# flxrcz/hommx

Hardware: AMD Instinct MI355X
Metric: micro-cell solves/sec (higher is better)
Workload: dtype f64

## Files before the change

### hommx_amd/csrc/fused2d.hip

```cpp
#include <hip/hip_runtime.h>
#include <stdint.h>

#include <type_traits>

#include "kernels.h"
#include "sweep_acc.h"

#ifndef HOMMX_FUSED_WAVES_PER_SIMD
#define HOMMX_FUSED_WAVES_PER_SIMD 2
#endif

namespace hommx {

typedef double d4 __attribute__((ext_vector_type(4)));
typedef double d2 __attribute__((ext_vector_type(2)));

__device__ __forceinline__ double uniform_f64(double v) {
  return __hiloint2double(__builtin_amdgcn_readfirstlane(__double2hiint(v)),
                          __builtin_amdgcn_readfirstlane(__double2loint(v)));
}

struct CoefRow {
  double a0, a1;
  double a0m, a1m;
};

constexpr int MATP = 48;

template <int NB>
struct alignas(16) Lds {
  double mat[(NB + 1) * MATP];
  double ubuf[4 * NB];
  double tsc[16 * 17];
  double rrow[2][NB];
  double vrow[2][NB];
  double vnat[2][NB];
  double e0row[NB];
  double e1row[NB];
  double e0nat[NB];
  double e1nat[NB];
  double dgnat[NB];
  double cenat[NB + 2];
};

struct NoFact {};
template <int NB, bool FACT>
__global__ __launch_bounds__(64, HOMMX_FUSED_WAVES_PER_SIMD) void k_poisson2d_fused(
    const double* __restrict__ coef, const double* __restrict__ Mmat, double* __restrict__ out,
    int32_t* __restrict__ info, int n, long long ncells, const CoefSource src, std::conditional_t<FACT, double*, NoFact> fact
#ifdef HOMMX_FUSED_DEBUG
    , double* __restrict__ dbg
#endif
) {
  constexpr int NT = NB / 16, KK = NB / 4, CG = 64 / NB;
  constexpr int P = MATP;
  __shared__ Lds<NB> L;

  const long long cell = blockIdx.x;
  if (cell >= ncells) return;
  __builtin_assume(n >= 3);
  __builtin_assume(n <= NB);
  const int l = threadIdx.x;
  const int j = l & 15, k = l >> 4;
  const int c = l % NB, g = l / NB;
  const int lb = l - c;
  const int p0 = NB - n;
  const bool valid = c >= p0;
  const int cn = c - p0;
  const int cm = valid ? (c == p0 ? NB - 1 : c - 1) : c;
  const int cp = valid ? (c == NB - 1 ? p0 : c + 1) : c;
  const int prow = (c & 3) * KK + (c >> 2);

  const int ownB = (k + 1) * P + j;
  int leftB[NT];
#pragma unroll
  for (int tj = 0; tj < NT; ++tj) {
    const int col = 16 * tj + j;
    leftB[tj] = (k + 1) * P + (col == p0 ? NB - 1 : col - 1);
  }
#define OWN(ti, tj, r) (ownB + (16 * (ti) + 4 * (r)) * P + 16 * (tj))
#define LEFT(ti, tj, r) (leftB[tj] + (16 * (ti) + 4 * (r)) * P)
  const unsigned matOff = accl::lds_offset(&L.mat[0]);
  const unsigned haloA = matOff + 8u * (unsigned)(p0 * P + j);

  const int mode = src.mode;
  const unsigned char* mask = static_cast<const unsigned char*>(src.table);
  const double* table = static_cast<const double*>(src.table);
  const double* cc = mode == COEF_STREAM ? coef + cell * (2ll * n * n) : coef + cell * 2;
  constexpr int NL = NB * NB / 64;
  double2 pv[NL];
  if (mode == COEF_STREAM) {
#pragma unroll
    for (int i = 0; i < NL; ++i) {
      const int el = 2 * l + 128 * i;
      pv[i] = el < 2 * n * n ? *reinterpret_cast<const double2*>(cc + el) : double2{0.0, 0.0};
    }
  }

  for (int i = l; i < (NB + 1) * P; i += 64) L.mat[i] = 0.0;
  if (l == 0) L.cenat[0] = 0.0;

  double m00 = 1.0, m01 = 0.0, m10 = 0.0, m11 = 1.0;
  if (Mmat) {
    const double* mp = Mmat + cell * 4;
    m00 = mp[0]; m01 = mp[1]; m10 = mp[2]; m11 = mp[3];
  }
  const double al = uniform_f64(0.5 * (m00 * m00 + m10 * m10));
  const double be = uniform_f64(0.5 * (m01 * m01 + m11 * m11));
  const double ga = uniform_f64(0.5 * (m00 * m01 + m10 * m11));
  const double ab = uniform_f64(al - 2.0 * ga + be);

  double ph0 = 0.0, ph1 = 0.0;
  if (mode != COEF_STREAM) {
    ph0 = cc[0];
    ph1 = cc[1];
  }
  const int nq = src.nq;
  auto sample = [&](long long el) {
    double acc = 0.0;
    for (int q = 0; q < nq; ++q)
      acc = add_rn(acc, mul_rn(src.weights[q], div_rn(1.0, add_rn(ph0, mul_rn(ph1, table[el * nq + q])))));
    return acc;
  };
  auto load_pair = [&](long long el, double& a0, double& a1) {
    if (mode == COEF_TWO_PHASE) {
      const uchar2 mk = *reinterpret_cast<const uchar2*>(mask + el);
      a0 = mk.x ? ph1 : ph0;
      a1 = mk.y ? ph1 : ph0;
    } else if (mode == COEF_AFFINE) {
      const double2 g2 = *reinterpret_cast<const double2*>(table + el);
      a0 = add_rn(ph0, mul_rn(ph1, g2.x));
      a1 = add_rn(ph0, mul_rn(ph1, g2.y));
    } else if (mode == COEF_RECIPROCAL) {
      a0 = sample(el);
      a1 = sample(el + 1);
    } else {
      const double2 v = *reinterpret_cast<const double2*>(cc + el);
      a0 = v.x; a1 = v.y;
    }
  };
  int esh;
  {
    int ef = 0;
    if (mode == COEF_STREAM) {
      int hm = 0;
#pragma unroll
      for (int i = 0; i < NL; ++i) hm = max(hm, max(__double2hiint(pv[i].x) & 0x7fffffff, __double2hiint(pv[i].y) & 0x7fffffff));
      ef = hm >> 20;
    } else {
      for (long long el = 2 * l; el < 2ll * n * n; el += 128) {
        double a0, a1;
        load_pair(el, a0, a1);
        const int f0 = (__double2hiint(a0) >> 20) & 0x7ff, f1 = (__double2hiint(a1) >> 20) & 0x7ff;
        ef = max(ef, max(f0, f1));
      }
    }
#pragma unroll
    for (int off = 32; off >= 1; off >>= 1) ef = max(ef, __shfl_xor(ef, off, 64));
    const int fm = (__double2hiint(6.0 * (al + be)) >> 20) & 0x7ff;
    const int sh = (ef == 0 || ef == 0x7ff ? 0 : ef - 1023) + (fm == 0 || fm == 0x7ff ? 0 : fm - 1023) + 2;
    esh = __builtin_amdgcn_readfirstlane(ef == 0 || ef == 0x7ff ? 0 : sh);
  }
  auto load_row = [&](int jc) {
    CoefRow r;
    r.a0 = 0.0; r.a1 = 0.0;
    if (valid) {
      load_pair(2 * (jc * n + cn), r.a0, r.a1);
      r.a0 = ldexp(r.a0, -esh);
      r.a1 = ldexp(r.a1, -esh);
    }
    r.a0m = __shfl(r.a0, lb + cm, 64);
    r.a1m = __shfl(r.a1, lb + cm, 64);
    return r;
  };
  auto st_diag = [&](const CoefRow& cur, const CoefRow& prev) {
    return valid ? cur.a0 * al + cur.a1 * be + cur.a0m * ab + prev.a0m * be + prev.a1m * al + prev.a1 * ab : 1.0;
  };
  auto st_E = [&](const CoefRow& cur, const CoefRow& prev) { return (cur.a0 + prev.a1) * (ga - al); };
  auto st_N = [&](const CoefRow& cur) { return (cur.a1 + cur.a0m) * (ga - be); };
  auto st_NE = [&](const CoefRow& cur) { return -ga * (cur.a0 + cur.a1); };
  auto st_p0 = [&](const CoefRow& cur, const CoefRow& prev) { return cur.a0 - cur.a0m - prev.a1m + prev.a1; };
  auto st_p1 = [&](const CoefRow& cur, const CoefRow& prev) { return cur.a1 + cur.a0m - prev.a0m - prev.a1; };

  auto band_write = [&](double dv, double ov, bool sym, bool clear) {
    if (g == 0) {
      const double d_ = clear ? 0.0 : dv, o_ = clear ? 0.0 : ov;
      L.mat[(c + 1) * P + c] = d_;
      if (valid) {
        L.mat[(cp + 1) * P + c] = o_;
        if (sym) L.mat[(c + 1) * P + cp] = o_;
      }
    }
  };

  [[maybe_unused]] double* rec = nullptr;
  if constexpr (FACT) rec = fact + cell * fused_fact_doubles(n);
  [[maybe_unused]] double* srec = nullptr;
  if constexpr (FACT) srec = rec + fused_fact_header(NB);

  double wf[NT][KK];
  double a[NT][NT][4];
  d4 slr[NT][NT];
  double rr[2];
  double rlm;
  CoefRow cur;
  double asum;
  __syncthreads();
  {
    const CoefRow rowA = load_row(n - 2);
    const CoefRow rowB = load_row(n - 1);
    cur = load_row(0);
    asum = (rowB.a0 + rowB.a1) + (cur.a0 + cur.a1);
    if constexpr (FACT) {
      const double neB = st_NE(rowB);
      const double c1 = __shfl(neB, lb + cm, 64);
      if (g == 0) {
        rec[c] = st_N(rowB);
        rec[NB + c] = c1;
      }
      if (l < 4) rec[4 * NB + l] = l == 0 ? m00 : l == 1 ? m01 : l == 2 ? m10 : m11;
      if (l == 4) rec[4 * NB + 4] = (double)esh;
    }
    {
      const double dv = st_diag(rowB, rowA), ov = st_E(rowB, rowA);
      band_write(dv, ov, true, false);
      __syncthreads();
#pragma unroll
      for (int ti = 0; ti < NT; ++ti)
#pragma unroll
        for (int tj = 0; tj <= ti; ++tj)
#pragma unroll
          for (int r = 0; r < 4; ++r) slr[ti][tj][r] = L.mat[OWN(ti, tj, r)];
      __syncthreads();
      band_write(dv, ov, true, true);
      __syncthreads();
    }
    {
      const double dv = st_N(rowB), ov = st_NE(rowB);
      band_write(dv, ov, false, false);
      __syncthreads();
#pragma unroll
      for (int t = 0; t < NT; ++t)
#pragma unroll
        for (int kk = 0; kk < KK; ++kk) wf[t][kk] = L.mat[OWN(kk >> 2, t, kk & 3)];
      __syncthreads();
      band_write(dv, ov, false, true);
      __syncthreads();
    }
    {
      const double dv = -st_diag(cur, rowB), ov = -st_E(cur, rowB);
      band_write(dv, ov, true, false);
      __syncthreads();
#pragma unroll
      for (int ti = 0; ti < NT; ++ti)
#pragma unroll
        for (int tj = 0; tj < NT; ++tj)
#pragma unroll
          for (int r = 0; r < 4; ++r) a[ti][tj][r] = L.mat[OWN(ti, tj, r)];
      __syncthreads();
      band_write(dv, ov, true, true);
      __syncthreads();
    }
    rr[0] = st_p0(cur, rowB); rr[1] = st_p1(cur, rowB);
    rlm = (k >> 1) ? st_p1(rowB, rowA) : st_p0(rowB, rowA);
  }
  double ga_ = 0.0, gb_ = 0.0;
  int bad = 0, badstep = 0;
  double wselR[NT];
#pragma unroll
  for (int tj = 0; tj < NT; ++tj) wselR[tj] = (k == 3 && 16 * tj + j == p0) ? 1.0 : 0.0;
  const double wselC = (j == 15 && k == (p0 & 3)) ? 1.0 : 0.0;
  double indw[KK];
#pragma unroll
  for (int q = 0; q < KK; ++q) indw[q] = uniform_f64((q == (p0 >> 2)) ? 1.0 : 0.0);

  for (int jr = 0; jr <= n - 2; ++jr) {
    const bool lastStep = (jr == n - 2);
    CoefRow nxt = cur;
    if (!lastStep) {
      nxt = load_row(jr + 1);
      asum += nxt.a0 + nxt.a1;
    }
    const double e0c = st_N(cur);
    const double neC = st_NE(cur);
    const double e1c = __shfl(neC, lb + cm, 64);
    if (lastStep) {
      for (int i = l; i < (NB + 1) * P; i += 64) L.mat[i] = 0.0;
      __syncthreads();
      if (g == 0) {
        L.mat[(c + 1) * P + c] = e0c;
        if (valid) L.mat[(c + 1) * P + cp] = neC;
      }
      __syncthreads();
#pragma unroll
      for (int t = 0; t < NT; ++t)
#pragma unroll
        for (int kk = 0; kk < KK; ++kk) wf[t][kk] += L.mat[OWN(kk >> 2, t, kk & 3)];
      __syncthreads();
    }
    const double dgc = st_diag(nxt, cur), cec = st_E(nxt, cur);
    if (g == 0) {
      L.rrow[0][prow] = rr[0];
      L.rrow[1][prow] = rr[1];
      L.e0row[prow] = e0c;
      L.e1row[prow] = e1c;
      L.e0nat[c] = e0c;
      L.e1nat[c] = e1c;
      L.dgnat[c] = dgc;
      L.cenat[1 + c] = cec;
    }

    {
      int badj = 0;
#ifdef HOMMX_FUSED_SWEEP32
      accl::Sweep<NB>::run(a, L.ubuf, j, k, badj);
#else
      __builtin_amdgcn_s_setprio(1);
      if constexpr (NB == 32) accl::block_inverse32(a, L.ubuf, L.tsc, j, k, badj);
      else accl::Sweep<NB>::run(a, L.ubuf, j, k, badj);
      __builtin_amdgcn_s_setprio(0);
#endif
      if (badj && !bad) { bad = 1; badstep = jr + 1; }
    }
    if constexpr (FACT) {
#pragma unroll
      for (int ti = 0; ti < NT; ++ti)
#pragma unroll
        for (int tj = 0; tj < NT; ++tj)
#pragma unroll
          for (int r = 0; r < 4; ++r) srec[((ti * NT + tj) * 4 + r) * 64 + l] = a[ti][tj][r];
      if (g == 0) {
        srec[NB * NB + 2 * NB + c] = e0c;
        srec[NB * NB + 3 * NB + c] = e1c;
      }
    }
#ifdef HOMMX_FUSED_DEBUG
    if (dbg && cell == 0) {
      double* q = dbg + (size_t)jr * 4 * NB * NB;
#pragma unroll
      for (int ti = 0; ti < NT; ++ti)
#pragma unroll
        for (int tj = 0; tj < NT; ++tj)
#pragma unroll
          for (int r = 0; r < 4; ++r) q[(16 * ti + 4 * r + k) * NB + 16 * tj + j] = a[ti][tj][r];
#pragma unroll
      for (int t = 0; t < NT; ++t)
#pragma unroll
        for (int kk = 0; kk < KK; ++kk) q[NB * NB + (16 * t + j) * NB + 4 * kk + k] = wf[t][kk];
    }
#endif

    if (!lastStep) {
#pragma unroll
      for (int ti = 0; ti < NT; ++ti)
#pragma unroll
        for (int tj = 0; tj < NT; ++tj)
#pragma unroll
          for (int r = 0; r < 4; ++r) L.mat[OWN(ti, tj, r)] = a[ti][tj][r];
#pragma unroll
      for (int tj = 0; tj < NT; ++tj)
        accl::masked_lds_store<accl::RowMask<3>::lo, accl::RowMask<3>::hi>(haloA + 128u * tj, a[NT - 1][tj][3]);
    }

    d4 vt[NT][NT];
#pragma unroll
    for (int x = 0; x < NT; ++x)
#pragma unroll
      for (int y = 0; y < NT; ++y) vt[x][y] = d4{0.0, 0.0, 0.0, 0.0};
#pragma unroll
    for (int kk = 0; kk < KK; ++kk)
#pragma unroll
      for (int x = 0; x < NT; ++x)
#pragma unroll
        for (int y = 0; y < NT; ++y)
          vt[x][y] = __builtin_amdgcn_mfma_f64_16x16x4f64(a[kk >> 2][x][kk & 3], wf[y][kk], vt[x][y], 0, 0, 0);

#pragma unroll
    for (int kk = 0; kk < KK; ++kk)
#pragma unroll
      for (int x = 0; x < NT; ++x)
#pragma unroll
        for (int y = 0; y <= x; ++y)
          slr[x][y] = __builtin_amdgcn_mfma_f64_16x16x4f64(vt[kk >> 2][x][kk & 3], wf[y][kk], slr[x][y], 0, 0, 0);

    double z;
    {
      double part[2][NT];
#pragma unroll
      for (int m = 0; m < 2; ++m)
#pragma unroll
        for (int tj = 0; tj < NT; ++tj) part[m][tj] = 0.0;
#pragma unroll
      for (int m = 0; m < 2; ++m)
#pragma unroll
        for (int ti = 0; ti < NT; ++ti) {
          const d4 q = *reinterpret_cast<const d4*>(&L.rrow[m][k * KK + 4 * ti]);
#pragma unroll
          for (int r = 0; r < 4; ++r)
#pragma unroll
            for (int tj = 0; tj < NT; ++tj) part[m][tj] = fma(q[r], a[ti][tj][r], part[m][tj]);
        }
      if (NT == 2) {
        double s_[2];
#pragma unroll
        for (int m = 0; m < 2; ++m) {
          double x = part[m][0], y = part[m][NT - 1];
          swap16(x, y);
          s_[m] = x + y;
        }
        swap32(s_[0], s_[1]);
        z = s_[0] + s_[1];
      } else {
        double x = part[0][0], y = part[1][0];
        swap32(x, y);
        z = add_xor16(x + y);
      }
    }
    ga_ = fma(z, rr[0], ga_);
    gb_ = fma(z, rr[1], gb_);
    L.vnat[k >> 1][c] = z;
    L.vrow[k >> 1][prow] = z;
    if constexpr (FACT) {
      if (NB == 32 || !(k & 1)) srec[NB * NB + (k >> 1) * NB + c] = z;
      srec += fused_fact_step(NB);
    }

    {
      double part[2][NT];
#pragma unroll
      for (int m = 0; m < 2; ++m) {
        double v[KK];
#pragma unroll
        for (int q4 = 0; q4 < KK; q4 += 4) {
          const d4 q = *reinterpret_cast<const d4*>(&L.vrow[m][k * KK + q4]);
          v[q4] = q[0]; v[q4 + 1] = q[1]; v[q4 + 2] = q[2]; v[q4 + 3] = q[3];
        }
#pragma unroll
        for (int t = 0; t < NT; ++t) {
          double acc = 0.0;
#pragma unroll
          for (int kk = 0; kk < KK; ++kk) acc = fma(v[kk], wf[t][kk], acc);
          part[m][t] = acc;
        }
      }
      double z6;
      if (NT == 2) {
        double s_[2];
#pragma unroll
        for (int m = 0; m < 2; ++m) {
          double x = part[m][0], y = part[m][NT - 1];
          swap16(x, y);
          s_[m] = x + y;
        }
        swap32(s_[0], s_[1]);
        z6 = s_[0] + s_[1];
      } else {
        double x = part[0][0], y = part[1][0];
        swap32(x, y);
        z6 = add_xor16(x + y);
      }
      rlm += z6;
    }

    if (!lastStep) {
      double e0r[KK], e1r[KK];
#pragma unroll
      for (int q4 = 0; q4 < KK; q4 += 4) {
        const d4 x = *reinterpret_cast<const d4*>(&L.e0row[k * KK + q4]);
        const d4 y = *reinterpret_cast<const d4*>(&L.e1row[k * KK + q4]);
        e0r[q4] = x[0]; e0r[q4 + 1] = x[1]; e0r[q4 + 2] = x[2]; e0r[q4 + 3] = x[3];
        e1r[q4] = y[0]; e1r[q4 + 1] = y[1]; e1r[q4 + 2] = y[2]; e1r[q4 + 3] = y[3];
      }
      {
        double e0q[NT], e1q[NT], dgq[NT], ceq[NT], cemq[NT];
#pragma unroll
        for (int tj = 0; tj < NT; ++tj) {
          e0q[tj] = L.e0nat[16 * tj + j];
          e1q[tj] = L.e1nat[16 * tj + j];
          dgq[tj] = L.dgnat[16 * tj + j];
          ceq[tj] = L.cenat[1 + 16 * tj + j];
          cemq[tj] = L.cenat[16 * tj + j];
        }
#pragma unroll
        for (int ti = 0; ti < NT; ++ti)
#pragma unroll
          for (int r = 0; r < 4; ++r)
#pragma unroll
            for (int tj = 0; tj < NT; ++tj) {
              const double nl = L.mat[LEFT(ti, tj, r)];
              const double nu = L.mat[OWN(ti, tj, r) - P];
              const double nul = L.mat[LEFT(ti, tj, r) - P];
              const double x = fma(e1q[tj], nl, e0q[tj] * a[ti][tj][r]);
              const double xu = fma(e1q[tj], nul, e0q[tj] * nu);
              a[ti][tj][r] = -fma(e0r[4 * ti + r], x, e1r[4 * ti + r] * xu);
            }
#pragma unroll
        for (int t = 0; t < NT; ++t) {
          using namespace accl;
#define DIAG_LO(r) (OneLane<0, 4 * (r)>::lo | OneLane<1, 4 * (r) + 1>::lo | OneLane<2, 4 * (r) + 2>::lo | OneLane<3, 4 * (r) + 3>::lo)
#define DIAG_HI(r) (OneLane<0, 4 * (r)>::hi | OneLane<1, 4 * (r) + 1>::hi | OneLane<2, 4 * (r) + 2>::hi | OneLane<3, 4 * (r) + 3>::hi)
          masked_sub4<DIAG_LO(0), DIAG_HI(0), DIAG_LO(1), DIAG_HI(1), DIAG_LO(2), DIAG_HI(2), DIAG_LO(3), DIAG_HI(3)>(
              a[t][t][0], a[t][t][1], a[t][t][2], a[t][t][3], dgq[t]);
#define SUB_LO(r) (((r) ? OneLane<0, (4 * (r) - 1) & 15>::lo : 0u) | OneLane<1, 4 * (r)>::lo | OneLane<2, 4 * (r) + 1>::lo | OneLane<3, 4 * (r) + 2>::lo)
#define SUB_HI(r) (((r) ? OneLane<0, (4 * (r) - 1) & 15>::hi : 0u) | OneLane<1, 4 * (r)>::hi | OneLane<2, 4 * (r) + 1>::hi | OneLane<3, 4 * (r) + 2>::hi)
          masked_sub4<SUB_LO(0), SUB_HI(0), SUB_LO(1), SUB_HI(1), SUB_LO(2), SUB_HI(2), SUB_LO(3), SUB_HI(3)>(
              a[t][t][0], a[t][t][1], a[t][t][2], a[t][t][3], ceq[t]);
#define SUP_LO(r) (OneLane<0, 4 * (r) + 1>::lo | OneLane<1, 4 * (r) + 2>::lo | OneLane<2, 4 * (r) + 3>::lo | ((r) < 3 ? OneLane<3, (4 * (r) + 4) & 15>::lo : 0u))
#define SUP_HI(r) (OneLane<0, 4 * (r) + 1>::hi | OneLane<1, 4 * (r) + 2>::hi | OneLane<2, 4 * (r) + 3>::hi | ((r) < 3 ? OneLane<3, (4 * (r) + 4) & 15>::hi : 0u))
          masked_sub4<SUP_LO(0), SUP_HI(0), SUP_LO(1), SUP_HI(1), SUP_LO(2), SUP_HI(2), SUP_LO(3), SUP_HI(3)>(
              a[t][t][0], a[t][t][1], a[t][t][2], a[t][t][3], cemq[t]);
#undef DIAG_LO
#undef DIAG_HI
#undef SUB_LO
#undef SUB_HI
#undef SUP_LO
#undef SUP_HI
        }
        if (NT == 2) {
          using namespace accl;
          masked_sub<OneLane<0, 15>::lo, OneLane<0, 15>::hi>(a[NT - 1][0][0], ceq[0]);
          masked_sub<OneLane<3, 0>::lo, OneLane<3, 0>::hi>(a[0][NT - 1][3], cemq[NT - 1]);
        }
        {
          const double cw = readlane_f64(cec, NB - 1);
#pragma unroll
          for (int tj = 0; tj < NT; ++tj) a[NT - 1][tj][3] = fma(-cw, wselR[tj], a[NT - 1][tj][3]);
          const double vcol = -cw * wselC;
#pragma unroll
          for (int ti = 0; ti < NT; ++ti)
#pragma unroll
            for (int r = 0; r < 4; ++r) a[ti][NT - 1][r] = fma(vcol, indw[4 * ti + r], a[ti][NT - 1][r]);
        }
      }

#pragma unroll
      for (int x = 0; x < NT; ++x)
#pragma unroll
        for (int y = 0; y < NT; ++y)
#pragma unroll
          for (int r = 0; r < 4; ++r) L.mat[OWN(x, y, r)] = vt[x][y][r];
#pragma unroll
      for (int y = 0; y < NT; ++y)
        accl::masked_lds_store<accl::RowMask<3>::lo, accl::RowMask<3>::hi>(haloA + 128u * y, vt[NT - 1][y][3]);
#pragma unroll
      for (int t = 0; t < NT; ++t)
#pragma unroll
        for (int kk = 0; kk < KK; ++kk) {
          const double up = L.mat[OWN(kk >> 2, t, kk & 3) - P];
          wf[t][kk] = fma(e1r[kk], up, e0r[kk] * vt[kk >> 2][t][kk & 3]);
        }

      {
        const double v0 = L.vnat[0][c], v1 = L.vnat[1][c];
        const double vm0 = L.vnat[0][cm], vm1 = L.vnat[1][cm];
        rr[0] = fma(vm0, e1c, fma(v0, e0c, st_p0(nxt, cur)));
        rr[1] = fma(vm1, e1c, fma(v1, e0c, st_p1(nxt, cur)));
      }
      cur = nxt;
      __syncthreads();
    }
  }

  {
    if (NT == 2) {
#pragma unroll
      for (int r = 0; r < 4; ++r) L.mat[OWN(1, 0, r)] = slr[NT - 1][0][r];
      __syncthreads();
    }
#pragma unroll
    for (int ti = 0; ti < NT; ++ti)
#pragma unroll
      for (int tj = 0; tj < NT; ++tj)
#pragma unroll
        for (int r = 0; r < 4; ++r) {
          if (tj <= ti) a[ti][tj][r] = -slr[ti][tj][r];
          else a[ti][tj][r] = -L.mat[(16 + j + 1) * P + 4 * r + k];
        }
    {
      using namespace accl;
#pragma unroll
      for (int tj = 0; tj < NT; ++tj) amov<RowMask<3>::lo, RowMask<3>::hi>(a[NT - 1][tj][3], 0.0);
#pragma unroll
      for (int ti = 0; ti < NT; ++ti)
#pragma unroll
        for (int r = 0; r < 4; ++r) amov<ColMask<15>::lo, ColMask<15>::hi>(a[ti][NT - 1][r], 0.0);
      amov<OneLane<3, 15>::lo, OneLane<3, 15>::hi>(a[NT - 1][NT - 1][3], -1.0);
    }
    if (c == NB - 1) rlm = 0.0;
    __syncthreads();
    L.rrow[k >> 1][prow] = rlm;
    L.vnat[k >> 1][c] = rlm;
    __syncthreads();
    int badj = 0;
    accl::Sweep<NB>::run(a, L.ubuf, j, k, badj);
    if (badj && !bad) { bad = 1; badstep = n; }
    if constexpr (FACT) {
#pragma unroll
      for (int ti = 0; ti < NT; ++ti)
#pragma unroll
        for (int tj = 0; tj < NT; ++tj)
#pragma unroll
          for (int r = 0; r < 4; ++r) srec[((ti * NT + tj) * 4 + r) * 64 + l] = a[ti][tj][r];
    }
    double part[2][NT];
#pragma unroll
    for (int m = 0; m < 2; ++m)
#pragma unroll
      for (int tj = 0; tj < NT; ++tj) part[m][tj] = 0.0;
#pragma unroll
    for (int m = 0; m < 2; ++m)
#pragma unroll
      for (int ti = 0; ti < NT; ++ti) {
        const d4 q = *reinterpret_cast<const d4*>(&L.rrow[m][k * KK + 4 * ti]);
#pragma unroll
        for (int r = 0; r < 4; ++r)
#pragma unroll
          for (int tj = 0; tj < NT; ++tj) part[m][tj] = fma(q[r], a[ti][tj][r], part[m][tj]);
      }
    double z;
    if (NT == 2) {
      double s_[2];
#pragma unroll
      for (int m = 0; m < 2; ++m) {
        double x = part[m][0], y = part[m][NT - 1];
        swap16(x, y);
        s_[m] = x + y;
      }
      swap32(s_[0], s_[1]);
      z = s_[0] + s_[1];
    } else {
      double x = part[0][0], y = part[1][0];
      swap32(x, y);
      z = add_xor16(x + y);
    }
    ga_ = fma(z, L.vnat[0][c], ga_);
    gb_ = fma(z, L.vnat[1][c], gb_);
    if constexpr (FACT) {
      if (NB == 32 || !(k & 1)) rec[2 * NB + (k >> 1) * NB + c] = z;
    }
  }

  double g00 = (k < 2) ? ga_ : 0.0, g01 = (k < 2) ? gb_ : 0.0, g11 = (k < 2) ? 0.0 : gb_;
#pragma unroll
  for (int off = 32; off >= 1; off >>= 1) {
    g00 += __shfl_xor(g00, off, 64);
    g01 += __shfl_xor(g01, off, 64);
    g11 += __shfl_xor(g11, off, 64);
    asum += __shfl_xor(asum, off, 64);
  }
  if (l == 0) {
    const double h = 1.0 / n;
    constexpr int DUP = 32 / NB;
    const double sc = 0.25 * h * h / DUP;
    const double c0 = 0.5 * h * h * asum / CG;
    const double t00 = m00 * g00 + m01 * g01, t01 = m00 * g01 + m01 * g11;
    const double t10 = m10 * g00 + m11 * g01, t11 = m10 * g01 + m11 * g11;
    double* o = out + cell * 4;
    o[0] = ldexp(c0 + sc * (t00 * m00 + t01 * m01), esh);
    o[1] = ldexp(sc * (t00 * m10 + t01 * m11), esh);
    o[2] = ldexp(sc * (t10 * m00 + t11 * m01), esh);
    o[3] = ldexp(c0 + sc * (t10 * m10 + t11 * m11), esh);
    if (info) info[cell] = bad ? badstep : 0;
  }
#undef OWN
#undef LEFT
}

#ifndef HOMMX_FUSED_FACT_TU
hipError_t launch_poisson2d_fused(const double* d_coef, const double* d_M, double* d_out, int32_t* d_info,
                                  int n, long long ncells, hipStream_t stream, CoefSource src) {
  if (ncells <= 0) return hipSuccess;
  dim3 grid((unsigned)ncells), block(64);
#ifndef HOMMX_DEV_LDS_PAD
#define HOMMX_DEV_LDS_PAD 0
#endif
#ifdef HOMMX_FUSED_DEBUG
  extern double* g_fused_dbg;
  if (n <= 16)
    hipLaunchKernelGGL((k_poisson2d_fused<16, false>), grid, block, 0, stream, d_coef, d_M, d_out, d_info, n, ncells, src, NoFact{}, g_fused_dbg);
  else
    hipLaunchKernelGGL((k_poisson2d_fused<32, false>), grid, block, 0, stream, d_coef, d_M, d_out, d_info, n, ncells, src, NoFact{}, g_fused_dbg);
#else
  if (n <= 16)
    hipLaunchKernelGGL((k_poisson2d_fused<16, false>), grid, block, HOMMX_DEV_LDS_PAD, stream, d_coef, d_M, d_out, d_info, n, ncells, src, NoFact{});
  else
    hipLaunchKernelGGL((k_poisson2d_fused<32, false>), grid, block, HOMMX_DEV_LDS_PAD, stream, d_coef, d_M, d_out, d_info, n, ncells, src, NoFact{});
#endif
  return hipGetLastError();
}

#else
hipError_t launch_poisson2d_fused_fact(const double* d_coef, const double* d_M, double* d_out, int32_t* d_info, int n, long long ncells,
                                       hipStream_t stream, double* d_fact) {
  if (ncells <= 0) return hipSuccess;
  dim3 grid((unsigned)ncells), block(64);
  const CoefSource src;
#ifdef HOMMX_FUSED_DEBUG
  extern double* g_fused_dbg;
  if (n <= 16)
    hipLaunchKernelGGL((k_poisson2d_fused<16, true>), grid, block, 0, stream, d_coef, d_M, d_out, d_info, n, ncells, src, d_fact, g_fused_dbg);
  else
    hipLaunchKernelGGL((k_poisson2d_fused<32, true>), grid, block, 0, stream, d_coef, d_M, d_out, d_info, n, ncells, src, d_fact, g_fused_dbg);
#else
  if (n <= 16)
    hipLaunchKernelGGL((k_poisson2d_fused<16, true>), grid, block, 0, stream, d_coef, d_M, d_out, d_info, n, ncells, src, d_fact);
  else
    hipLaunchKernelGGL((k_poisson2d_fused<32, true>), grid, block, 0, stream, d_coef, d_M, d_out, d_info, n, ncells, src, d_fact);
#endif
  return hipGetLastError();
}
#endif

}
```

### hommx_amd/csrc/kernels.h

```cpp
#pragma once
#include <hip/hip_runtime.h>
#include <stdint.h>

#include <type_traits>

#include "../../include/hommx_hip.h"

namespace hommx {

struct KindSizes {
  int bs, t, n_comp;
};
constexpr KindSizes kind_sizes(int dim, int kind) {
  const int te = dim * (dim + 1) / 2;
  return kind == HOMMX_KIND_POISSON_SCALAR   ? KindSizes{1, dim, 1}
         : kind == HOMMX_KIND_POISSON_MATRIX ? KindSizes{1, dim, te}
         : kind == HOMMX_KIND_ELASTICITY_ISO ? KindSizes{dim, te, 2}
                                             : KindSizes{dim, te, te * (te + 1) / 2};
}

template <typename F>
auto dispatch_dim_kind(int dim, int kind, F&& f) {
  auto with_dim = [&](auto D) {
    switch (kind) {
      case 0: return f(D, std::integral_constant<int, 0>{});
      case 1: return f(D, std::integral_constant<int, 1>{});
      case 2: return f(D, std::integral_constant<int, 2>{});
      default: return f(D, std::integral_constant<int, 3>{});
    }
  };
  return dim == 2 ? with_dim(std::integral_constant<int, 2>{}) : with_dim(std::integral_constant<int, 3>{});
}

__device__ __forceinline__ double mul_rn(double a, double b) {
#pragma clang fp contract(off)
  return a * b;
}
__device__ __forceinline__ double add_rn(double a, double b) {
#pragma clang fp contract(off)
  return a + b;
}
__device__ __forceinline__ double div_rn(double a, double b) {
#pragma clang fp contract(off)
  return a / b;
}
enum CoefMode { COEF_STREAM = 0, COEF_TWO_PHASE = 1, COEF_AFFINE = 2, COEF_RECIPROCAL = 3 };
struct CoefSource {
  int mode = COEF_STREAM;
  int nq = 0;
  const void* table = nullptr;
  const double* weights = nullptr;
};

hipError_t launch_poisson2d_fused(const double* d_coef, const double* d_M, double* d_out, int32_t* d_info,
                                  int n, long long ncells, hipStream_t stream, CoefSource src = CoefSource());

constexpr long long fused_fact_header(int NB) { return 4 * NB + 8; }
constexpr long long fused_fact_step(int NB) { return (long long)NB * NB + 4 * NB; }
constexpr long long fused_fact_doubles(int n) {
  return fused_fact_header(n <= 16 ? 16 : 32) + (n - 1) * fused_fact_step(n <= 16 ? 16 : 32) + (n <= 16 ? 16 * 16 : 32 * 32);
}
hipError_t launch_poisson2d_fused_fact(const double* d_coef, const double* d_M, double* d_out, int32_t* d_info, int n, long long ncells,
                                       hipStream_t stream, double* d_fact);
hipError_t launch_fused2d_subst(const double* d_fact, double* d_corr, int n, long long ncells, hipStream_t stream);
hipError_t launch_fused2d_subst_rhs(const double* d_fact, const double* d_P, int n_loads, bool per_cell, const double* d_M, double* d_corr, int n,
                                    long long ncells, hipStream_t stream);

hipError_t launch_expand_separable(CoefSource src, const double* d_params, double* d_coef, long long n_el, int n_comp, long long ncells,
                                   hipStream_t stream);

hipError_t launch_expand_two_phase(const unsigned char* d_mask, const double* d_values, double* d_coef, long long n_el,
                                   int n_comp, long long ncells, hipStream_t stream);

struct ReconArgs {
  int n = 0;
  double vol_struct = 0.0;
  long long ndof = 0, n_el = 0;
  const int32_t* el_nodes = nullptr;
  const double* grads = nullptr;
  const double* vol = nullptr;
  const double* corr = nullptr;
  const double* coef = nullptr;
  const double* M = nullptr;
  const double* xi = nullptr;
  double* stats = nullptr;
  double* strain = nullptr;
  double* flux = nullptr;
  double* slot = nullptr;
  int n_regions = 0;
  const uint8_t* region = nullptr;
  double* region_stats = nullptr;
};
size_t recon_lds_limit();
hipError_t launch_reconstruct(const ReconArgs& a, int dim, int kind, bool mesh, long long nc, hipStream_t stream);

struct SensArgs {
  int n = 0;
  double vol_struct = 0.0;
  long long ndof = 0, n_el = 0;
  const int32_t* el_nodes = nullptr;
  const double* grads = nullptr;
  const double* vol = nullptr;
  const double* corr = nullptr;
  const double* M = nullptr;
  int n_dirs = 0;
  bool per_cell = false;
  const double* dirs = nullptr;
  double* dA = nullptr;
  const double* weights = nullptr;
  double* grad = nullptr;
};
hipError_t launch_sensitivity(const SensArgs& a, int dim, int kind, bool mesh, long long nc, hipStream_t stream);

struct LoadArgs {
  int n = 0;
  double vol_struct = 0.0;
  long long ndof = 0, n_el = 0;
  const int32_t* el_nodes = nullptr;
  const double* grads = nullptr;
  const double* vol = nullptr;
  const double* corr = nullptr;
  const double* coef = nullptr;
  const double* M = nullptr;
  int n_loads = 0;
  bool per_cell = false;
  const double* P = nullptr;
  double* P_eff = nullptr;
  double* energy = nullptr;
  double* stats = nullptr;
  double* strain = nullptr;
  double* flux = nullptr;
};
hipError_t launch_polar(const LoadArgs& a, int dim, int kind, bool mesh, long long nc, hipStream_t stream);
hipError_t launch_load_stats(const LoadArgs& a, int dim, int kind, bool mesh, long long nc, hipStream_t stream);

struct LoadOverride {
  const double* P = nullptr;
  int n_loads = 0;
  bool per_cell = false;
};

hipError_t run_fp64_calibration(double* mfma_flops_per_s, double* fma_flops_per_s, double* mfma_lds_fed_flops_per_s = nullptr);

}

namespace hommx {
struct BlockedWorkspace;
int blocked_workspace_create(BlockedWorkspace** out, int dim, int n, int kind);
void blocked_workspace_destroy(BlockedWorkspace* ws);
int blocked_solve(BlockedWorkspace* ws, long long ncells, const double* d_coef, const double* d_M,
                  double* d_out, int32_t* d_info, hipStream_t stream, double* d_corr = nullptr, const LoadOverride* loads = nullptr);
int blocked_reserve(BlockedWorkspace* ws, long long n_cells);
const char* blocked_route_name(const BlockedWorkspace* ws);
const char* blocked_route_detail(BlockedWorkspace* ws);
const char* blocked_corrector_route_name(const BlockedWorkspace* ws);
double blocked_flops_per_cell(const BlockedWorkspace* ws);
}
```

Baseline: 6.996 million.

## Add isotropic specialization of fused 2D Poisson kernel when no metric matrix

Adds an ISO template parameter used when no per-cell metric matrix is supplied. In that case the off-diagonal stencil coupling (NE term) vanishes, so the kernel skips the neighbour-coupling LDS traffic, the halo stores, the shuffles and the extra FMAs in the Schur update, and computes the updates as pure diagonal scalings. The specialization is compiled in a separate translation unit, and the general launcher dispatches to it when d_M is null. It relies on ga=0 being exact for the identity metric.

```diff
diff --git a/hommx_amd/csrc/fused2d.hip b/hommx_amd/csrc/fused2d.hip
--- a/hommx_amd/csrc/fused2d.hip
+++ b/hommx_amd/csrc/fused2d.hip
@@ -44,7 +44,7 @@
 };
 
 struct NoFact {};
-template <int NB, bool FACT>
+template <int NB, bool FACT, bool ISO>
 __global__ __launch_bounds__(64, HOMMX_FUSED_WAVES_PER_SIMD) void k_poisson2d_fused(
     const double* __restrict__ coef, const double* __restrict__ Mmat, double* __restrict__ out,
     int32_t* __restrict__ info, int n, long long ncells, const CoefSource src, std::conditional_t<FACT, double*, NoFact> fact
@@ -54,6 +54,7 @@
 ) {
   constexpr int NT = NB / 16, KK = NB / 4, CG = 64 / NB;
   constexpr int P = MATP;
+  static_assert(!(FACT && ISO), "the factor record keeps the general path");
   __shared__ Lds<NB> L;
 
   const long long cell = blockIdx.x;
@@ -72,7 +73,7 @@
   const int prow = (c & 3) * KK + (c >> 2);
 
   const int ownB = (k + 1) * P + j;
-  int leftB[NT];
+  [[maybe_unused]] int leftB[NT];
 #pragma unroll
   for (int tj = 0; tj < NT; ++tj) {
     const int col = 16 * tj + j;
@@ -81,7 +82,7 @@
 #define OWN(ti, tj, r) (ownB + (16 * (ti) + 4 * (r)) * P + 16 * (tj))
 #define LEFT(ti, tj, r) (leftB[tj] + (16 * (ti) + 4 * (r)) * P)
   const unsigned matOff = accl::lds_offset(&L.mat[0]);
-  const unsigned haloA = matOff + 8u * (unsigned)(p0 * P + j);
+  [[maybe_unused]] const unsigned haloA = matOff + 8u * (unsigned)(p0 * P + j);
 
   const int mode = src.mode;
   const unsigned char* mask = static_cast<const unsigned char*>(src.table);
@@ -101,14 +102,14 @@
   if (l == 0) L.cenat[0] = 0.0;
 
   double m00 = 1.0, m01 = 0.0, m10 = 0.0, m11 = 1.0;
-  if (Mmat) {
+  if (!ISO && Mmat) {
     const double* mp = Mmat + cell * 4;
     m00 = mp[0]; m01 = mp[1]; m10 = mp[2]; m11 = mp[3];
   }
-  const double al = uniform_f64(0.5 * (m00 * m00 + m10 * m10));
-  const double be = uniform_f64(0.5 * (m01 * m01 + m11 * m11));
-  const double ga = uniform_f64(0.5 * (m00 * m01 + m10 * m11));
-  const double ab = uniform_f64(al - 2.0 * ga + be);
+  const double al = ISO ? 0.5 : uniform_f64(0.5 * (m00 * m00 + m10 * m10));
+  const double be = ISO ? 0.5 : uniform_f64(0.5 * (m01 * m01 + m11 * m11));
+  const double ga = ISO ? 0.0 : uniform_f64(0.5 * (m00 * m01 + m10 * m11));
+  const double ab = ISO ? 1.0 : uniform_f64(al - 2.0 * ga + be);
 
   double ph0 = 0.0, ph1 = 0.0;
   if (mode != COEF_STREAM) {
@@ -282,14 +283,19 @@
       asum += nxt.a0 + nxt.a1;
     }
     const double e0c = st_N(cur);
-    const double neC = st_NE(cur);
-    const double e1c = __shfl(neC, lb + cm, 64);
+    [[maybe_unused]] double neC = 0.0, e1c = 0.0;
+    if constexpr (!ISO) {
+      neC = st_NE(cur);
+      e1c = __shfl(neC, lb + cm, 64);
+    }
     if (lastStep) {
       for (int i = l; i < (NB + 1) * P; i += 64) L.mat[i] = 0.0;
       __syncthreads();
       if (g == 0) {
         L.mat[(c + 1) * P + c] = e0c;
-        if (valid) L.mat[(c + 1) * P + cp] = neC;
+        if constexpr (!ISO) {
+          if (valid) L.mat[(c + 1) * P + cp] = neC;
+        }
       }
       __syncthreads();
 #pragma unroll
@@ -303,9 +309,9 @@
       L.rrow[0][prow] = rr[0];
       L.rrow[1][prow] = rr[1];
       L.e0row[prow] = e0c;
-      L.e1row[prow] = e1c;
+      if constexpr (!ISO) L.e1row[prow] = e1c;
       L.e0nat[c] = e0c;
-      L.e1nat[c] = e1c;
+      if constexpr (!ISO) L.e1nat[c] = e1c;
       L.dgnat[c] = dgc;
       L.cenat[1 + c] = cec;
     }
@@ -350,7 +356,7 @@
     }
 #endif
 
-    if (!lastStep) {
+    if (!ISO && !lastStep) {
 #pragma unroll
       for (int ti = 0; ti < NT; ++ti)
 #pragma unroll
@@ -463,20 +469,27 @@
     }
 
     if (!lastStep) {
-      double e0r[KK], e1r[KK];
+      double e0r[KK];
+      [[maybe_unused]] double e1r[KK];
 #pragma unroll
       for (int q4 = 0; q4 < KK; q4 += 4) {
-        const d4 x = *reinterpret_cast<const d4*>(&L.e0row[k * KK + q4]);
-        const d4 y = *reinterpret_cast<const d4*>(&L.e1row[k * KK + q4]);
-        e0r[q4] = x[0]; e0r[q4 + 1] = x[1]; e0r[q4 + 2] = x[2]; e0r[q4 + 3] = x[3];
-        e1r[q4] = y[0]; e1r[q4 + 1] = y[1]; e1r[q4 + 2] = y[2]; e1r[q4 + 3] = y[3];
+        if constexpr (ISO) {
+          const d4 x = *reinterpret_cast<const d4*>(&L.e0row[k * KK + q4]);
+          e0r[q4] = x[0]; e0r[q4 + 1] = x[1]; e0r[q4 + 2] = x[2]; e0r[q4 + 3] = x[3];
+        } else {
+          const d4 x = *reinterpret_cast<const d4*>(&L.e0row[k * KK + q4]);
+          const d4 y = *reinterpret_cast<const d4*>(&L.e1row[k * KK + q4]);
+          e0r[q4] = x[0]; e0r[q4 + 1] = x[1]; e0r[q4 + 2] = x[2]; e0r[q4 + 3] = x[3];
+          e1r[q4] = y[0]; e1r[q4 + 1] = y[1]; e1r[q4 + 2] = y[2]; e1r[q4 + 3] = y[3];
+        }
       }
       {
-        double e0q[NT], e1q[NT], dgq[NT], ceq[NT], cemq[NT];
+        double e0q[NT], dgq[NT], ceq[NT], cemq[NT];
+        [[maybe_unused]] double e1q[NT];
 #pragma unroll
         for (int tj = 0; tj < NT; ++tj) {
           e0q[tj] = L.e0nat[16 * tj + j];
-          e1q[tj] = L.e1nat[16 * tj + j];
+          if constexpr (!ISO) e1q[tj] = L.e1nat[16 * tj + j];
           dgq[tj] = L.dgnat[16 * tj + j];
           ceq[tj] = L.cenat[1 + 16 * tj + j];
           cemq[tj] = L.cenat[16 * tj + j];
@@ -487,12 +500,16 @@
           for (int r = 0; r < 4; ++r)
 #pragma unroll
             for (int tj = 0; tj < NT; ++tj) {
-              const double nl = L.mat[LEFT(ti, tj, r)];
-              const double nu = L.mat[OWN(ti, tj, r) - P];
-              const double nul = L.mat[LEFT(ti, tj, r) - P];
-              const double x = fma(e1q[tj], nl, e0q[tj] * a[ti][tj][r]);
-              const double xu = fma(e1q[tj], nul, e0q[tj] * nu);
-              a[ti][tj][r] = -fma(e0r[4 * ti + r], x, e1r[4 * ti + r] * xu);
+              if constexpr (ISO) {
+                a[ti][tj][r] = -(e0r[4 * ti + r] * (e0q[tj] * a[ti][tj][r]));
+              } else {
+                const double nl = L.mat[LEFT(ti, tj, r)];
+                const double nu = L.mat[OWN(ti, tj, r) - P];
+                const double nul = L.mat[LEFT(ti, tj, r) - P];
+                const double x = fma(e1q[tj], nl, e0q[tj] * a[ti][tj][r]);
+                const double xu = fma(e1q[tj], nul, e0q[tj] * nu);
+                a[ti][tj][r] = -fma(e0r[4 * ti + r], x, e1r[4 * ti + r] * xu);
+              }
             }
 #pragma unroll
         for (int t = 0; t < NT; ++t) {
@@ -533,28 +550,40 @@
         }
       }
 
-#pragma unroll
-      for (int x = 0; x < NT; ++x)
+      if constexpr (ISO) {
+#pragma unroll
+        for (int t = 0; t < NT; ++t)
+#pragma unroll
+          for (int kk = 0; kk < KK; ++kk) wf[t][kk] = e0r[kk] * vt[kk >> 2][t][kk & 3];
+      } else {
+#pragma unroll
+        for (int x = 0; x < NT; ++x)
+#pragma unroll
+          for (int y = 0; y < NT; ++y)
+#pragma unroll
+            for (int r = 0; r < 4; ++r) L.mat[OWN(x, y, r)] = vt[x][y][r];
 #pragma unroll
         for (int y = 0; y < NT; ++y)
-#pragma unroll
-          for (int r = 0; r < 4; ++r) L.mat[OWN(x, y, r)] = vt[x][y][r];
-#pragma unroll
-      for (int y = 0; y < NT; ++y)
-        accl::masked_lds_store<accl::RowMask<3>::lo, accl::RowMask<3>::hi>(haloA + 128u * y, vt[NT - 1][y][3]);
-#pragma unroll
-      for (int t = 0; t < NT; ++t)
-#pragma unroll
-        for (int kk = 0; kk < KK; ++kk) {
-          const double up = L.mat[OWN(kk >> 2, t, kk & 3) - P];
-          wf[t][kk] = fma(e1r[kk], up, e0r[kk] * vt[kk >> 2][t][kk & 3]);
-        }
+          accl::masked_lds_store<accl::RowMask<3>::lo, accl::RowMask<3>::hi>(haloA + 128u * y, vt[NT - 1][y][3]);
+#pragma unroll
+        for (int t = 0; t < NT; ++t)
+#pragma unroll
+          for (int kk = 0; kk < KK; ++kk) {
+            const double up = L.mat[OWN(kk >> 2, t, kk & 3) - P];
+            wf[t][kk] = fma(e1r[kk], up, e0r[kk] * vt[kk >> 2][t][kk & 3]);
+          }
+      }
 
       {
         const double v0 = L.vnat[0][c], v1 = L.vnat[1][c];
-        const double vm0 = L.vnat[0][cm], vm1 = L.vnat[1][cm];
-        rr[0] = fma(vm0, e1c, fma(v0, e0c, st_p0(nxt, cur)));
-        rr[1] = fma(vm1, e1c, fma(v1, e0c, st_p1(nxt, cur)));
+        if constexpr (ISO) {
+          rr[0] = fma(v0, e0c, st_p0(nxt, cur));
+          rr[1] = fma(v1, e0c, st_p1(nxt, cur));
+        } else {
+          const double vm0 = L.vnat[0][cm], vm1 = L.vnat[1][cm];
+          rr[0] = fma(vm0, e1c, fma(v0, e0c, st_p0(nxt, cur)));
+          rr[1] = fma(vm1, e1c, fma(v1, e0c, st_p1(nxt, cur)));
+        }
       }
       cur = nxt;
       __syncthreads();
@@ -666,26 +695,45 @@
 #undef LEFT
 }
 
-#ifndef HOMMX_FUSED_FACT_TU
-hipError_t launch_poisson2d_fused(const double* d_coef, const double* d_M, double* d_out, int32_t* d_info,
-                                  int n, long long ncells, hipStream_t stream, CoefSource src) {
-  if (ncells <= 0) return hipSuccess;
-  dim3 grid((unsigned)ncells), block(64);
 #ifndef HOMMX_DEV_LDS_PAD
 #define HOMMX_DEV_LDS_PAD 0
 #endif
 #ifdef HOMMX_FUSED_DEBUG
-  extern double* g_fused_dbg;
+extern double* g_fused_dbg;
+#define HOMMX_FUSED_LDS 0
+#define HOMMX_FUSED_DBG_ARG , g_fused_dbg
+#else
+#define HOMMX_FUSED_LDS HOMMX_DEV_LDS_PAD
+#define HOMMX_FUSED_DBG_ARG
+#endif
+
+#if defined(HOMMX_FUSED_ISO_TU)
+hipError_t launch_poisson2d_fused_iso(const double* d_coef, double* d_out, int32_t* d_info, int n, long long ncells, hipStream_t stream,
+                                      CoefSource src) {
+  if (ncells <= 0) return hipSuccess;
+  dim3 grid((unsigned)ncells), block(64);
+  const double* d_M = nullptr;
   if (n <= 16)
-    hipLaunchKernelGGL((k_poisson2d_fused<16, false>), grid, block, 0, stream, d_coef, d_M, d_out, d_info, n, ncells, src, NoFact{}, g_fused_dbg);
+    hipLaunchKernelGGL((k_poisson2d_fused<16, false, true>), grid, block, HOMMX_FUSED_LDS, stream, d_coef, d_M, d_out, d_info, n, ncells, src,
+                       NoFact{} HOMMX_FUSED_DBG_ARG);
   else
-    hipLaunchKernelGGL((k_poisson2d_fused<32, false>), grid, block, 0, stream, d_coef, d_M, d_out, d_info, n, ncells, src, NoFact{}, g_fused_dbg);
-#else
+    hipLaunchKernelGGL((k_poisson2d_fused<32, false, true>), grid, block, HOMMX_FUSED_LDS, stream, d_coef, d_M, d_out, d_info, n, ncells, src,
+                       NoFact{} HOMMX_FUSED_DBG_ARG);
+  return hipGetLastError();
+}
+
+#elif !defined(HOMMX_FUSED_FACT_TU)
+hipError_t launch_poisson2d_fused(const double* d_coef, const double* d_M, double* d_out, int32_t* d_info,
+                                  int n, long long ncells, hipStream_t stream, CoefSource src) {
+  if (ncells <= 0) return hipSuccess;
+  if (!d_M) return launch_poisson2d_fused_iso(d_coef, d_out, d_info, n, ncells, stream, src);
+  dim3 grid((unsigned)ncells), block(64);
   if (n <= 16)
-    hipLaunchKernelGGL((k_poisson2d_fused<16, false>), grid, block, HOMMX_DEV_LDS_PAD, stream, d_coef, d_M, d_out, d_info, n, ncells, src, NoFact{});
+    hipLaunchKernelGGL((k_poisson2d_fused<16, false, false>), grid, block, HOMMX_FUSED_LDS, stream, d_coef, d_M, d_out, d_info, n, ncells, src,
+                       NoFact{} HOMMX_FUSED_DBG_ARG);
   else
-    hipLaunchKernelGGL((k_poisson2d_fused<32, false>), grid, block, HOMMX_DEV_LDS_PAD, stream, d_coef, d_M, d_out, d_info, n, ncells, src, NoFact{});
-#endif
+    hipLaunchKernelGGL((k_poisson2d_fused<32, false, false>), grid, block, HOMMX_FUSED_LDS, stream, d_coef, d_M, d_out, d_info, n, ncells, src,
+                       NoFact{} HOMMX_FUSED_DBG_ARG);
   return hipGetLastError();
 }
 
@@ -695,18 +743,12 @@
   if (ncells <= 0) return hipSuccess;
   dim3 grid((unsigned)ncells), block(64);
   const CoefSource src;
-#ifdef HOMMX_FUSED_DEBUG
-  extern double* g_fused_dbg;
   if (n <= 16)
-    hipLaunchKernelGGL((k_poisson2d_fused<16, true>), grid, block, 0, stream, d_coef, d_M, d_out, d_info, n, ncells, src, d_fact, g_fused_dbg);
+    hipLaunchKernelGGL((k_poisson2d_fused<16, true, false>), grid, block, 0, stream, d_coef, d_M, d_out, d_info, n, ncells, src,
+                       d_fact HOMMX_FUSED_DBG_ARG);
   else
-    hipLaunchKernelGGL((k_poisson2d_fused<32, true>), grid, block, 0, stream, d_coef, d_M, d_out, d_info, n, ncells, src, d_fact, g_fused_dbg);
-#else
-  if (n <= 16)
-    hipLaunchKernelGGL((k_poisson2d_fused<16, true>), grid, block, 0, stream, d_coef, d_M, d_out, d_info, n, ncells, src, d_fact);
-  else
-    hipLaunchKernelGGL((k_poisson2d_fused<32, true>), grid, block, 0, stream, d_coef, d_M, d_out, d_info, n, ncells, src, d_fact);
-#endif
+    hipLaunchKernelGGL((k_poisson2d_fused<32, true, false>), grid, block, 0, stream, d_coef, d_M, d_out, d_info, n, ncells, src,
+                       d_fact HOMMX_FUSED_DBG_ARG);
   return hipGetLastError();
 }
 #endif
diff --git a/hommx_amd/csrc/fused2d_iso.hip b/hommx_amd/csrc/fused2d_iso.hip
--- /dev/null
+++ b/hommx_amd/csrc/fused2d_iso.hip
@@ -0,0 +1,2 @@
+#define HOMMX_FUSED_ISO_TU
+#include "fused2d.hip"
diff --git a/hommx_amd/csrc/kernels.h b/hommx_amd/csrc/kernels.h
--- a/hommx_amd/csrc/kernels.h
+++ b/hommx_amd/csrc/kernels.h
@@ -54,6 +54,8 @@
 
 hipError_t launch_poisson2d_fused(const double* d_coef, const double* d_M, double* d_out, int32_t* d_info,
                                   int n, long long ncells, hipStream_t stream, CoefSource src = CoefSource());
+hipError_t launch_poisson2d_fused_iso(const double* d_coef, double* d_out, int32_t* d_info, int n, long long ncells, hipStream_t stream,
+                                      CoefSource src);
 
 constexpr long long fused_fact_header(int NB) { return 4 * NB + 8; }
 constexpr long long fused_fact_step(int NB) { return (long long)NB * NB + 4 * NB; }
```

Result: faster. 7.916 million (median of 6 runs) (+13.1%).
